# OpenMined/PIR

Measured on NVIDIA B200. Metric: pir_queries_per_sec, higher is better.
Workload: dtype u64

## Files before the change

pir_b200/csrc/context.cu:

```cuda
#include <atomic>
#include <cmath>
#include <cstdio>
#include <cstdlib>
#include <cstring>
#include <map>
#include <memory>
#include <optional>
#include <string>
#include <tuple>
#include <vector>

#include "../../include/pir_b200.h"
#include "behz_host.h"
#include "host_math.h"
#include "kernels.cuh"

using namespace pirb;

namespace {

thread_local std::string g_err;
int fail(int code, const std::string& msg) {
  g_err = msg;
  return code;
// ... 392 lines not shown
    n_rows = (u32)((npt + dimL - 1) / dimL);
    u64 off = compact_rows ? compact_rows : c->dims[0];
    for (int e = 1; e < d - 1; ++e) off += c->dims[e];
    sv_last = d_sv + off * ctL;
  }
  int n_split;
  RC(run_scan(c, sv_last, sv_qstride, n_queries, dimL, n_rows, npt, d >= 2, &n_split, st, svt));
  if (prof) cudaEventRecord(c->ev[3], st);
  if (d == 1) {
    if (partial) {
      LAUNCH(c, launch_modadd_reduce(P, c->part.p, ctL, n_split, d_out, 1, st, n_queries, (u64)n_split * ctL, ctL));
    } else {
      LAUNCH(c, launch_ntt_inv(P, c->part.p, d_out, 2 * k, k, 0, n_split, (u64)n_rows * ctL, n_queries,
                               (u64)n_split * n_rows * ctL, ctL, st));
    }
    if (prof) { cudaEventRecord(c->ev[4], st); cudaEventRecord(c->ev[5], st); }
    return 0;
  }
  RC(c->bufA[0].ensure((size_t)n_queries * n_rows * ctL * sizeof(u64)));
  LAUNCH(c, launch_ntt_inv(P, c->part.p, c->bufA[0].p, (int)(n_rows * 2 * k), k, 0, n_split, (u64)n_rows * ctL,
                           n_queries, (u64)n_split * n_rows * ctL, (u64)n_rows * ctL, st));
  if (prof) cudaEventRecord(c->ev[4], st);
  if (forked) CU(cudaStreamWaitEvent(st, c->ev_join, 0));
  u32 n_entries = n_rows;
  u32 w = 1;
  int cur = 0;
  for (int l = d - 2; l >= 0; --l) {
    const u32 dim = (l == 0) ? (c->top_hi - c->top_lo) : c->dims[l];
    const u32 n_groups = (n_entries + dim - 1) / dim;
    const u32 w_out = w * c->two_er;
    u64 sv_off = (l == 0) ? (compact_rows ? 0 : c->top_lo) : (compact_rows ? compact_rows : c->dims[0]);
    for (int e = 1; e < l; ++e) sv_off += c->dims[e];
    const u64 n_cts_in = (u64)n_entries * w;
    RC(c->pts.ensure((size_t)n_queries * n_cts_in * c->two_er * c->ptL * sizeof(u64)));
    LAUNCH(c, launch_reencode_ntt(P, c->bufA[cur].p, c->pts.p, (int)(n_queries * n_cts_in), st));
    const u32 slices = (u32)(c->ptL / 256);
    const int ns = dim_mac_config(P, (u64)slices * w_out * n_groups * n_queries, dim, c->sm_count);
    RC(c->part.ensure((size_t)n_queries * ns * n_groups * w_out * ctL * sizeof(u64)));
    LAUNCH(c, launch_dim_mac(P, c->pts.p, n_cts_in * c->two_er * c->ptL, d_sv + sv_off * ctL, sv_qstride, n_queries, dim,
                             n_entries, n_groups, w_out, ns, c->part.p, st));
    const u64 lvl_cts = (u64)n_groups * w_out;
    if (l == 0 && partial) {
      LAUNCH(c, launch_modadd_reduce(P, c->part.p, lvl_cts * ctL, ns, d_out, lvl_cts, st, n_queries, (u64)ns * lvl_cts * ctL,
                                     lvl_cts * ctL));
    } else {
      u64* dst = d_out;
      if (l != 0) {
        RC(c->bufA[cur ^ 1].ensure((size_t)n_queries * lvl_cts * ctL * sizeof(u64)));
        dst = c->bufA[cur ^ 1].p;
      }
      LAUNCH(c, launch_ntt_inv(P, c->part.p, dst, (int)(lvl_cts * 2 * k), k, 0, ns, lvl_cts * ctL, n_queries,
                               (u64)ns * lvl_cts * ctL, lvl_cts * ctL, st));
    }
    n_entries = n_groups;
    w = w_out;
    cur ^= 1;
  }
  if (prof) cudaEventRecord(c->ev[5], st);
  return 0;
}

int ct_level(pirb_ctx* c, const u64* key, const u64* A, u64 a_bstride, int s1, const u64* S, u64 s_bstride, u32 dim,
             u32 n_entries, int n_queries, u64* out, u64 out_bstride, cudaStream_t st) {
  pirb_ctx::CtMul& M = c->ct;
  const DevParams& P = c->P;
  const BehzC& B = M.B;
  const int k = c->k, nb = M.nbsk, sp = s1 + 1;
  const u64 N = c->N;
  const u64 ctL = c->ctL;
  const u64 sq_stride = (u64)dim * ctL, sb_stride = (u64)dim * 2 * nb * N;
  RC(M.sq.ensure((size_t)n_queries * sq_stride * sizeof(u64)));
  RC(M.sb.ensure((size_t)n_queries * sb_stride * sizeof(u64)));
  LAUNCH(c, launch_ntt_fwd(P, S, M.sq.p, (int)(dim * 2 * k), k, 0, n_queries, s_bstride, sq_stride, st));
// ... 1410 lines not shown
```

pir_b200/csrc/kernels.cuh:

```cuda
#pragma once
#include <cuda_runtime.h>

#include "pirb_common.h"
#include "tc_plan.h"

namespace pirb {

struct LevelArgs {
  const u64* src_off;
  const u64* dst_off;
  int n_trees;
  int j;
  u32 ginv;
  u32 g;
  u64 q_stride;
  int n_queries;
  const u64* const* key_tab;
  u64* xch;
  u64* dbg;
  int dbg_clock;
};

cudaError_t launch_ntt_fwd(const DevParams& P, const u64* in, u64* out, int n_polys, int cycle, int off,
                           int n_batch, u64 in_bstride, u64 out_bstride, cudaStream_t st);
cudaError_t launch_ntt_inv(const DevParams& P, const u64* in, u64* out, int n_polys, int cycle, int off, int n_parts,
                           u64 part_stride, int n_batch, u64 in_bstride, u64 out_bstride, cudaStream_t st);

cudaError_t launch_db_preprocess(const DevParams& P, const u64* coeffs, u64* out, u64 n_pt, cudaStream_t st);

cudaError_t launch_ks_digits(const DevParams& P, const u64* work, const LevelArgs& L, u64* dig, cudaStream_t st);
cudaError_t launch_ks_mac_intt(const DevParams& P, const u64* dig, const u64* key, u64* acc, int n_nodes,
                               cudaStream_t st, const u64* const* key_tab = nullptr, u32 nodes_per_query = 1);
cudaError_t launch_ks_combine(const DevParams& P, u64* work, const LevelArgs& L, const u64* acc, int mode,
                              cudaStream_t st);

bool ks_cluster_supported(const DevParams& P);
cudaError_t launch_ks_level_cluster(const DevParams& P, u64* work, const LevelArgs& L, const u64* key, int mode,
                                    cudaStream_t st);

cudaError_t launch_mul_inv_pow_x(const DevParams& P, const u64* in, u64* out, u32 kpow, int n_cts, cudaStream_t st);

cudaError_t launch_scan(const DevParams& P, const u64* db, u64 num_pt, u32 dimL, u32 n_rows, const u64* sv,
                        u64 sv_qstride, int n_queries, int n_split, u64* part, cudaStream_t st);
void scan_config(const DevParams& P, u32 dimL, u32 n_rows, int n_queries, int sm_count, int* n_split);

cudaError_t launch_reencode_ntt(const DevParams& P, const u64* cts, u64* pts, int n_cts, cudaStream_t st);

int dim_mac_config(const DevParams& P, u64 base_ctas, u32 len, int sm_count);
cudaError_t launch_dim_mac(const DevParams& P, const u64* pts, u64 pts_qstride, const u64* sv, u64 sv_qstride,
                           int n_queries, u32 dim, u32 n_entries_in, u32 n_groups, u32 w_out, int n_split, u64* part,
                           cudaStream_t st);

cudaError_t launch_modadd_reduce(const DevParams& P, const u64* in, u64 stride, int n_parts, u64* out, u64 n_cts,
                                 cudaStream_t st, int n_batch = 1, u64 in_bstride = 0, u64 out_bstride = 0);
cudaError_t launch_modadd_reduce_ptrs(const DevParams& P, const u64* const* peers_dev, int n_parts, u64 offset_limbs,
                                      u64* out, u64 n_cts, cudaStream_t st);

cudaError_t launch_place_roots(const DevParams& P, const u64* query, u64 query_qstride, u64* work, const u64* root_off,
                               int n_trees, int n_queries, u64 q_stride, cudaStream_t st);

struct PushArgs {
  u64* const* peers;
  u32 n_ranks;
  u32 d0;
  u32 rows_per_rank;
  u64 slot_off;
  u64 g_first;
  u64 dst_qstride;
};
cudaError_t launch_ntt_fwd_push(const DevParams& P, const u64* in, u64 in_qstride, u32 n_entries, u32 n_queries,
                                const PushArgs& A, cudaStream_t st);
cudaError_t launch_push_head(const DevParams& P, const u64* in, u64 in_qstride, u32 n_entries, u32 n_queries,
                             const PushArgs& A, cudaStream_t st);
cudaError_t launch_push_rows(u64* const* peers_dev, u32 n_ranks, const u8* stage, u64 src_stride, u32 seg_bytes, u32 n_segs,
                             u64 dst_off, u64 dst_stride, cudaStream_t st);
cudaError_t launch_signal(u64* const* peers_dev, u32 n_ranks, u64 flag_off_limbs, u64 value, cudaStream_t st);
cudaError_t launch_wait(const u64* flags, u32 n_ranks, u64 value, u64 timeout_ns, u64* err, cudaStream_t st);

struct TcGeom {
// ... 46 lines not shown
```

pir_b200/csrc/kernels_ntt.cu:

```cuda
#include <cstdlib>
#include <set>
#include <type_traits>
#include <utility>

#include "kernels.cuh"
#include "pirb_device.cuh"

namespace pirb {

template <int LOGN>
struct Cfg {
  static constexpr int N = 1 << LOGN;
  static constexpr int NT = (N / 8 < 512) ? N / 8 : 512;
  static constexpr size_t SMEM = sizeof(u64) * N;
  static constexpr int MINB = LOGN <= 13 ? 2 : 1;
};

template <int LOGN, int ENG>
__global__ void __launch_bounds__(Cfg<LOGN>::NT, Cfg<LOGN>::MINB)
k_ntt_fwd(const __grid_constant__ DevParams P, const u64* __restrict__ in, u64* __restrict__ out, int cycle, int off,
          u64 in_bstride, u64 out_bstride) {
  constexpr int N = Cfg<LOGN>::N, NT = Cfg<LOGN>::NT;
  extern __shared__ u64 s[];
  const int tid = threadIdx.x;
// ... 224 lines not shown
           int n_parts, u64 part_stride, u64 in_bstride, u64 out_bstride) {
  constexpr int N = Cfg2<LOGN>::N, NT = Cfg2<LOGN>::NT;
  extern __shared__ u64 s[];
  const int tid = threadIdx.x;
  const int j = blockIdx.x % cycle;
  const u64 p0 = (u64)(blockIdx.x / cycle) * 2 * cycle + j;
  const ModC& m = P.m[j + off];
  double* TW = reinterpret_cast<double*>(s + 2 * N);
  u64* bar = s + 3 * N;
  ntt2_stage_table<LOGN, true>(m, TW, bar, tid);
  const u64* src = in + blockIdx.y * in_bstride + p0 * N;
  u64* dst = out + blockIdx.y * out_bstride + p0 * N;
#pragma unroll
  for (int i = tid; i < N; i += NT) {
    u64 v = src[i], w = src[(u64)cycle * N + i];
    for (int g = 1; g < n_parts; ++g) {
      v = addmod(v, src[g * part_stride + i], m.q);
      w = addmod(w, src[g * part_stride + (u64)cycle * N + i], m.q);
    }
    s[swz(i)] = eng_load<ENG_FP64>(v);
    s[N + swz(i)] = eng_load<ENG_FP64>(w);
  }
  __syncthreads();
  mbar_wait(bar, 0);
  ntt2_inverse<LOGN, NT>(s, TW, m, tid);
#pragma unroll
  for (int i = tid; i < N; i += NT) {
    dst[i] = eng_store_inv<ENG_FP64>(s[swz(i)], i, m);
    dst[(u64)cycle * N + i] = eng_store_inv<ENG_FP64>(s[N + swz(i)], i, m);
  }
}

template <int LOGN>
__global__ void __launch_bounds__(Cfg2<LOGN>::NT, 2)
k_reencode_ntt2(const __grid_constant__ DevParams P, const u64* __restrict__ cts, u64* __restrict__ pts) {
  constexpr int N = Cfg2<LOGN>::N, NT = Cfg2<LOGN>::NT;
  extern __shared__ u64 s[];
  const int tid = threadIdx.x;
  const int jp = blockIdx.z, e0 = blockIdx.y * 2;
  const u64 x = blockIdx.x;
  const int k = P.k;
  const ModC& m = P.m[jp];
  double* TW = reinterpret_cast<double*>(s + 2 * N);
  u64* bar = s + 3 * N;
  ntt2_stage_table<LOGN, false>(m, TW, bar, tid);
  const u64 mask = (u64)((1u << P.ptb) - 1);
  const u64 inc = m.q - P.t;
#pragma unroll
  for (int h = 0; h < 2; ++h) {
    const int e = e0 + h;
    const u64* src = cts + (x * 2 * k + (u64)P.re_poly[e] * k + P.re_mod[e]) * N;
    const u32 shift = P.re_shift[e];
#pragma unroll
    for (int i = tid; i < N; i += NT) {
      const u64 c = (src[i] >> shift) & mask;
      s[h * N + swz(i)] = eng_load<ENG_FP64>(c >= P.thr ? c + inc : c);
    }
  }
  __syncthreads();
  mbar_wait(bar, 0);
  ntt2_forward<LOGN, NT>(s, TW, m, tid);
#pragma unroll
  for (int h = 0; h < 2; ++h) {
    u64* dst = pts + ((x * P.two_er + e0 + h) * k + jp) * N;
#pragma unroll
    for (int i = tid; i < N; i += NT) dst[i] = eng_store_fwd<ENG_FP64>(s[h * N + swz(i)], m);
  }
}

static bool ntt2_ok(const DevParams& P) {
  static const bool off = getenv("PIRB_NTT2") && getenv("PIRB_NTT2")[0] == '0';
  return !off && P.ntt_engine == ENG_FP64 && P.logn <= 12 && P.logn >= 11;
}
template <typename K>
static cudaError_t ensure_smem2(K kernel, size_t bytes);

template <typename K>
static cudaError_t ensure_smem(K kernel, size_t bytes) {
  if (bytes <= 48 * 1024) return cudaSuccess;
  static std::set<std::pair<int, const void*>> configured;
  int dev = 0;
  cudaGetDevice(&dev);
  const auto key = std::make_pair(dev, reinterpret_cast<const void*>(kernel));
  if (configured.count(key)) return cudaSuccess;
  cudaError_t e = cudaFuncSetAttribute(kernel, cudaFuncAttributeMaxDynamicSharedMemorySize, (int)bytes);
  if (e == cudaSuccess) configured.insert(key);
  return e;
}

template <typename K>
static cudaError_t ensure_smem2(K kernel, size_t bytes) { return ensure_smem(kernel, bytes); }

template <int V>
using IntC = std::integral_constant<int, V>;

template <typename F>
static cudaError_t dispatch(const DevParams& P, F&& f) {
#define PIRB_CASE(LN)                                                   \
  case LN:                                                              \
    switch (P.ntt_engine) {                                             \
// ... 74 lines not shown
    kern<<<dim3((unsigned)n_pt, P.k), Cfg<LN>::NT, Cfg<LN>::SMEM, st>>>(P, coeffs, out);
    return cudaGetLastError();
  });
}

cudaError_t launch_ks_digits(const DevParams& P, const u64* work, const LevelArgs& L, u64* dig, cudaStream_t st) {
  const unsigned nodes = (unsigned)L.n_queries * L.n_trees << L.j;
  if (!nodes) return cudaSuccess;
  return dispatch(P, [&](auto ln, auto lz) {
    constexpr int LN = decltype(ln)::value;
    constexpr int LZ = decltype(lz)::value;
    auto kern = k_ks_digits<LN, LZ>;
    cudaError_t e = ensure_smem(kern, Cfg<LN>::SMEM);
    if (e != cudaSuccess) return e;
    kern<<<dim3(nodes, P.k + 1, P.k), Cfg<LN>::NT, Cfg<LN>::SMEM, st>>>(P, work, L, dig);
    return cudaGetLastError();
  });
}

cudaError_t launch_ks_mac_intt(const DevParams& P, const u64* dig, const u64* key, u64* acc, int n_nodes,
                               cudaStream_t st, const u64* const* key_tab, u32 nodes_per_query) {
  if (n_nodes <= 0) return cudaSuccess;
  return dispatch(P, [&](auto ln, auto lz) {
    constexpr int LN = decltype(ln)::value;
    constexpr int LZ = decltype(lz)::value;
    auto kern = k_ks_mac_intt<LN, LZ>;
    cudaError_t e = ensure_smem(kern, Cfg<LN>::SMEM);
    if (e != cudaSuccess) return e;
    kern<<<dim3(n_nodes, P.k + 1, 2), Cfg<LN>::NT, Cfg<LN>::SMEM, st>>>(P, dig, key, acc, key_tab, nodes_per_query);
    return cudaGetLastError();
  });
}

cudaError_t launch_reencode_ntt(const DevParams& P, const u64* cts, u64* pts, int n_cts, cudaStream_t st) {
  if (n_cts <= 0) return cudaSuccess;
  if (ntt2_ok(P) && P.two_er % 2 == 0) {
    auto go2 = [&](auto ln) -> cudaError_t {
      constexpr int LN = decltype(ln)::value;
      auto kern = k_reencode_ntt2<LN>;
      cudaError_t e = ensure_smem2(kern, Cfg2<LN>::SMEM);
      if (e != cudaSuccess) return e;
      kern<<<dim3(n_cts, P.two_er / 2, P.k), Cfg2<LN>::NT, Cfg2<LN>::SMEM, st>>>(P, cts, pts);
      return cudaGetLastError();
    };
    return P.logn == 12 ? go2(IntC<12>{}) : go2(IntC<11>{});
  }
  return dispatch(P, [&](auto ln, auto lz) {
    constexpr int LN = decltype(ln)::value;
    constexpr int LZ = decltype(lz)::value;
    auto kern = k_reencode_ntt<LN, LZ>;
    cudaError_t e = ensure_smem(kern, Cfg<LN>::SMEM);
    if (e != cudaSuccess) return e;
    kern<<<dim3(n_cts, P.two_er, P.k), Cfg<LN>::NT, Cfg<LN>::SMEM, st>>>(P, cts, pts);
    return cudaGetLastError();
  });
}

}
```

pir_b200/csrc/pirb_device.cuh:

```cuda
#pragma once
#include <cuda_runtime.h>

#include "pirb_common.h"

namespace pirb {

__device__ __forceinline__ u64 csub(u64 x, u64 q) { return x >= q ? x - q : x; }
__device__ __forceinline__ u64 addmod(u64 a, u64 b, u64 q) { return csub(a + b, q); }
__device__ __forceinline__ u64 submod(u64 a, u64 b, u64 q) { return a >= b ? a - b : a + q - b; }
__device__ __forceinline__ u64 negmod(u64 a, u64 q) { return a ? q - a : 0; }

__device__ __forceinline__ u64 shoup_lazy(u64 x, u64 w, u64 ws, u64 q) {
  u64 h = __umul64hi(x, ws);
  return x * w - h * q;
}
__device__ __forceinline__ u64 shoup(u64 x, u64 w, u64 ws, u64 q) { return csub(shoup_lazy(x, w, ws, q), q); }

__device__ __forceinline__ void mac128(u64& lo, u64& hi, u64 a, u64 b) {
  u64 pl = a * b, ph = __umul64hi(a, b);
  asm("add.cc.u64 %0, %0, %2;\n\taddc.u64 %1, %1, %3;" : "+l"(lo), "+l"(hi) : "l"(pl), "l"(ph));
}

__device__ __forceinline__ u64 barrett128(u64 lo, u64 hi, u64 q, u64 r_hi, u64 r_lo);
__device__ __forceinline__ double f64_modmul(double y, double w, double wi, double q);
// ... 229 lines not shown
  }
  ntt_inv_pass<LOGN, NT, 0, R0, LAZY>(s, m.irp, m.irps, q, tid);
  __syncthreads();
}

__device__ __forceinline__ u64 canon_fwd(u64 v, const ModC& m, bool lazy) {
  if (lazy) return barrett64(v, m.q, m.ratio_hi);
  v = v >= 2 * m.q ? v - 2 * m.q : v;
  return csub(v, m.q);
}
__device__ __forceinline__ u64 inv_finish(u64 v, const ModC& m) { return shoup(v, m.inv_n, m.inv_n_s, m.q); }

__device__ __forceinline__ double f64_modmul(double y, double w, double wi, double q) {
  const double M = 6755399441055744.0;
  const double h = __dmul_rn(y, w);
  const double l = __fma_rn(y, w, -h);
  const double c = __dadd_rn(__fma_rn(y, wi, M), -M);
  const double r = __fma_rn(-c, q, h);
  return __dadd_rn(r, l);
}
__device__ __forceinline__ double f64_canon(double v, double q, double qinv) {
  const double M = 6755399441055744.0;
  const double c = __dadd_rn(__fma_rn(v, qinv, M), -M);
  double r = __fma_rn(-c, q, v);
  return r < 0.0 ? __dadd_rn(r, q) : r;
}
__device__ __forceinline__ double u64_to_f64_exact(u64 v) {
  return __dadd_rn(__longlong_as_double((long long)(v | 0x4330000000000000ull)), -4503599627370496.0);
}
__device__ __forceinline__ u64 f64_to_u64_exact(double d) {
  return (u64)__double_as_longlong(__dadd_rn(d, 4503599627370496.0)) & 0x000FFFFFFFFFFFFFull;
}

struct TwGlobal {
  const double2* t;
  __device__ __forceinline__ void get(int i, double& w, double& wi) const {
    const double2 v = __ldg(t + i);
    w = v.x;
    wi = v.y;
  }
};
struct TwShared {
  const double* t;
  double qinv;
  __device__ __forceinline__ void get(int i, double& w, double& wi) const {
    w = t[i];
    wi = __dmul_rn(w, qinv);
  }
};

template <int LOGN, int NT, int S0, int R, class TW>
__device__ __forceinline__ void f64_fwd_pass(double* __restrict__ s, const TW tw, double q, int tid) {
  constexpr int N = 1 << LOGN;
  constexpr int E = 1 << R;
  constexpr int TL = N >> (S0 + R);
  constexpr int UNITS = N >> R;
#pragma unroll 1
  for (int u = tid; u < UNITS; u += NT) {
    const int lo = u & (TL - 1);
    const int hi = u / TL;
    const int base = hi * (TL << R) + lo;
    double x[E];
#pragma unroll
    for (int e = 0; e < E; ++e) x[e] = s[swz(base + e * TL)];
#pragma unroll
    for (int a = 0; a < R; ++a) {
      const int half = E >> (a + 1);
      const int mbase = (1 << (S0 + a)) + (hi << a);
#pragma unroll
      for (int b = 0; b < (1 << a); ++b) {
        double w, wi;
        tw.get(mbase + b, w, wi);
#pragma unroll
        for (int c = 0; c < half; ++c) {
          const int e0 = b * 2 * half + c, e1 = e0 + half;
          const double T = f64_modmul(x[e1], w, wi, q);
          x[e1] = __dadd_rn(x[e0], -T);
          x[e0] = __dadd_rn(x[e0], T);
        }
      }
    }
#pragma unroll
    for (int e = 0; e < E; ++e) s[swz(base + e * TL)] = x[e];
  }
}
template <int LOGN, int NT, int S0, int R, class TW>
__device__ __forceinline__ void f64_inv_pass(double* __restrict__ s, const TW iw, double q, int tid) {
  constexpr int N = 1 << LOGN;
  constexpr int E = 1 << R;
  constexpr int TL = N >> (S0 + R);
  constexpr int UNITS = N >> R;
#pragma unroll 1
  for (int u = tid; u < UNITS; u += NT) {
    const int lo = u & (TL - 1);
    const int hi = u / TL;
    const int base = hi * (TL << R) + lo;
    double x[E];
#pragma unroll
    for (int e = 0; e < E; ++e) x[e] = s[swz(base + e * TL)];
#pragma unroll
    for (int a = R - 1; a >= 0; --a) {
      const int dist = E >> (a + 1);
      const int g = dist * TL;
#pragma unroll
      for (int c = 0; c < dist; ++c) {
        double w, wi;
        iw.get(g + c * TL + lo, w, wi);
#pragma unroll
        for (int b = 0; b < (1 << a); ++b) {
          const int e0 = b * 2 * dist + c, e1 = e0 + dist;
          const double T = f64_modmul(x[e1], w, wi, q);
          x[e1] = __dadd_rn(x[e0], -T);
          x[e0] = __dadd_rn(x[e0], T);
        }
      }
    }
#pragma unroll
    for (int e = 0; e < E; ++e) s[swz(base + e * TL)] = x[e];
  }
}

enum { ENG_INT = 0, ENG_INT_LAZY = 1, ENG_FP64 = 2 };

template <int ENG>
__device__ __forceinline__ u64 eng_load(u64 v) {
  if constexpr (ENG == ENG_FP64) return (u64)__double_as_longlong(u64_to_f64_exact(v));
  else return v;
}
template <int ENG>
__device__ __forceinline__ u64 eng_store_fwd(u64 word, const ModC& m) {
  if constexpr (ENG == ENG_FP64) return f64_to_u64_exact(f64_canon(__longlong_as_double((long long)word), m.qd, m.qinv));
  else return canon_fwd(word, m, ENG == ENG_INT_LAZY);
}
template <int ENG>
__device__ __forceinline__ u64 eng_store_inv(u64 word, int i, const ModC& m) {
  if constexpr (ENG == ENG_FP64) {
    const double2 f2 = __ldg(m.fin + i);
    double t = f64_modmul(__longlong_as_double((long long)word), f2.x, f2.y, m.qd);
    t = t < 0.0 ? __dadd_rn(t, m.qd) : t;
    return f64_to_u64_exact(t);
  } else {
    return inv_finish(word, m);
  }
}
__device__ __forceinline__ double f64_addmod(double a, double b, double q) {
  const double s = __dadd_rn(a, b);
  return s >= q ? __dadd_rn(s, -q) : s;
}
__device__ __forceinline__ double f64_submod(double a, double b, double q) {
  const double d = __dadd_rn(a, -b);
  return d < 0.0 ? __dadd_rn(d, q) : d;
// ... 87 lines not shown
```

pir_b200/csrc/kernels_cluster.cu:

```cuda
#include <cooperative_groups.h>

#include <algorithm>
#include <cstdlib>

#include <type_traits>

#include "kernels.cuh"
#include "pirb_device.cuh"

namespace cg = cooperative_groups;

namespace pirb {

template <int LOGN>
struct CCfg {
  static constexpr int N = 1 << LOGN;
  static constexpr int NT = (N / 8 < 512) ? N / 8 : 512;
};

__device__ __forceinline__ u64 mod_down_c(u64 a, u64 last, const DevParams& P, int j, u64 Pq) {
  const ModC& m = P.m[j];
  u64 l = last + P.half_P;
  l = l >= Pq ? l - Pq : l;
  u64 r = submod(barrett64(l, m.q, m.ratio_hi), P.half_P_mod[j], m.q);
// ... 238 lines not shown
    }
  }
  PIRB_STAMP(7);
}

template <int LOGN, int K>
__global__ void __launch_bounds__(CCfg<LOGN>::NT, 2)
k_ks_level_cluster2(const __grid_constant__ DevParams P, u64* __restrict__ work, const LevelArgs L,
                    const u64* __restrict__ key_arg, int mode) {
  constexpr int N = CCfg<LOGN>::N, NT = CCfg<LOGN>::NT;
  constexpr int NB = K < 2 ? 2 : K;
  extern __shared__ u64 smem[];
  cg::cluster_group cluster = cg::this_cluster();
  const int tid = threadIdx.x;
  constexpr int k = K;
  const int I = (int)cluster.block_rank();
  const u32 z = blockIdx.x / (k + 1);
  const u32 kk = z & ((1u << L.j) - 1);
  const u32 tq = z >> L.j;
  const u32 ti = tq % L.n_trees, qi = tq / L.n_trees;
  const u64* __restrict__ key = L.key_tab ? L.key_tab[qi] : key_arg;
  const u64 ctL = (u64)2 * k * N;
  const u64* src = work + qi * L.q_stride + L.src_off[ti] + kk * ctL;
  const ModC& mI = P.m[I];
  const double qd = mI.qd, qinv = mI.qinv;
  double* TWb = reinterpret_cast<double*>(smem + (size_t)NB * N);
  u64* twbar = smem + (size_t)(NB + 1) * N;
  if (tid == 0) {
    mbar_init(twbar, 1);
    asm volatile("fence.mbarrier_init.release.cluster;" ::: "memory");
    mbar_expect_tx(twbar, N * 8);
    bulk_g2s_plain(TWb, mI.fw1, N * 8, twbar);
  }
  asm volatile("griddepcontrol.launch_dependents;");
  {
    constexpr int LINES = N * 8 / 128;
    for (int J = 0; J < k; ++J)
      for (int c = 0; c < 2; ++c) {
        const char* kp = reinterpret_cast<const char*>(key + ((u64)(J * 2 + c) * (k + 1) + I) * N);
        for (int l = tid; l < LINES; l += NT) asm volatile("prefetch.global.L2 [%0];" ::"l"(kp + (size_t)l * 128));
      }
    asm volatile("griddepcontrol.wait;" ::: "memory");
  }
#pragma unroll
  for (int J = 0; J < k; ++J) {
    u64* D = smem + (size_t)J * N;
    const u64* c1 = src + (u64)(k + J) * N;
    const u64 qJ = P.m[J].q;
    const bool need_reduce = qJ > mI.q;
#pragma unroll
    for (int i = tid; i < N; i += NT) {
      u64 v = c1[i];
      const u32 t = ((u32)i * L.g) & (2 * N - 1);
      if (t & N) v = negmod(v, qJ);
      if (need_reduce) v = barrett64(v, mI.q, mI.ratio_hi);
      D[swz(t & (N - 1))] = eng_load<ENG_FP64>(v);
    }
  }
  __syncthreads();
  mbar_wait(twbar, 0);
  {
    constexpr int R0 = ((LOGN - 1) % 3) + 1;
    const TwShared tw{TWb, qinv};
    auto pass_all = [&](auto s0, auto r) {
      constexpr int S0 = decltype(s0)::value, R = decltype(r)::value;
#pragma unroll
      for (int J = 0; J < k; ++J) f64_fwd_pass<LOGN, NT, S0, R>(reinterpret_cast<double*>(smem + (size_t)J * N), tw, qd, tid);
      __syncthreads();
    };
    pass_all(std::integral_constant<int, 0>{}, std::integral_constant<int, R0>{});
    if constexpr (LOGN > R0) pass_all(std::integral_constant<int, R0>{}, std::integral_constant<int, 3>{});
    if constexpr (LOGN > R0 + 3) pass_all(std::integral_constant<int, R0 + 3>{}, std::integral_constant<int, 3>{});
    if constexpr (LOGN > R0 + 6) pass_all(std::integral_constant<int, R0 + 6>{}, std::integral_constant<int, 3>{});
    if constexpr (LOGN > R0 + 9) pass_all(std::integral_constant<int, R0 + 9>{}, std::integral_constant<int, 3>{});
  }
  if (tid == 0) {
    asm volatile("fence.proxy.async.shared::cta;" ::: "memory");
    mbar_expect_tx(twbar, N * 8);
    bulk_g2s_plain(TWb, mI.iw1, N * 8, twbar);
  }
  {
    constexpr int CH = 4;
#pragma unroll 1
    for (int i0 = tid; i0 < N; i0 += CH * NT) {
      double a0[CH], a1[CH];
      int si[CH];
#pragma unroll
      for (int e = 0; e < CH; ++e) { si[e] = swz(i0 + e * NT); a0[e] = 0.0; a1[e] = 0.0; }
#pragma unroll
      for (int J = 0; J < k; ++J) {
        const u64* D = smem + (size_t)J * N;
        const u64* kp0 = key + ((u64)(J * 2 + 0) * (k + 1) + I) * N + i0;
        const u64* kp1 = key + ((u64)(J * 2 + 1) * (k + 1) + I) * N + i0;
        u64 dv[CH], k0[CH], k1[CH];
#pragma unroll
        for (int e = 0; e < CH; ++e) {
          dv[e] = D[si[e]];
          k0[e] = __ldg(kp0 + e * NT);
          k1[e] = __ldg(kp1 + e * NT);
        }
#pragma unroll
        for (int e = 0; e < CH; ++e) {
          const double y = __longlong_as_double((long long)dv[e]);
          const double kd0 = u64_to_f64_exact(k0[e]), kd1 = u64_to_f64_exact(k1[e]);
          a0[e] = __dadd_rn(a0[e], f64_modmul(y, kd0, __dmul_rn(kd0, qinv), qd));
          a1[e] = __dadd_rn(a1[e], f64_modmul(y, kd1, __dmul_rn(kd1, qinv), qd));
        }
      }
#pragma unroll
      for (int e = 0; e < CH; ++e) {
        smem[si[e]] = (u64)__double_as_longlong(a0[e]);
        (smem + N)[si[e]] = (u64)__double_as_longlong(a1[e]);
      }
    }
  }
  __syncthreads();
  mbar_wait(twbar, 1);
  {
    constexpr int R0 = ((LOGN - 1) % 3) + 1;
    const TwShared iw{TWb, qinv};
    auto pass_both = [&](auto s0, auto r) {
      constexpr int S0 = decltype(s0)::value, R = decltype(r)::value;
      f64_inv_pass<LOGN, NT, S0, R>(reinterpret_cast<double*>(smem), iw, qd, tid);
      f64_inv_pass<LOGN, NT, S0, R>(reinterpret_cast<double*>(smem + N), iw, qd, tid);
      __syncthreads();
    };
    if constexpr (LOGN > R0 + 9) pass_both(std::integral_constant<int, R0 + 9>{}, std::integral_constant<int, 3>{});
    if constexpr (LOGN > R0 + 6) pass_both(std::integral_constant<int, R0 + 6>{}, std::integral_constant<int, 3>{});
    if constexpr (LOGN > R0 + 3) pass_both(std::integral_constant<int, R0 + 3>{}, std::integral_constant<int, 3>{});
    if constexpr (LOGN > R0) pass_both(std::integral_constant<int, R0>{}, std::integral_constant<int, 3>{});
    pass_both(std::integral_constant<int, 0>{}, std::integral_constant<int, R0>{});
  }
  if (I == k) {
#pragma unroll
    for (int c = 0; c < 2; ++c) {
      u64* xo = L.xch + ((u64)z * 2 + c) * N;
      const u64* A = smem + (size_t)c * N;
#pragma unroll
      for (int i = tid; i < N; i += NT) xo[i] = eng_finish_inv_native<ENG_FP64>(A[swz(i)], i, mI);
    }
  } else {
#pragma unroll
    for (int c = 0; c < 2; ++c) {
      u64* A = smem + (size_t)c * N;
#pragma unroll
      for (int i = tid; i < N; i += NT) {
        const double2 f2 = __ldg(mI.fin + i);
        A[swz(i)] = (u64)__double_as_longlong(f64_modmul(__longlong_as_double((long long)A[swz(i)]), f2.x, f2.y, qd));
      }
    }
    const u64* sp = src + (u64)I * N;
    u64* SB = reinterpret_cast<u64*>(TWb);
#pragma unroll
    for (int i = tid; i < N; i += NT) SB[i] = sp[i];
  }
  cluster.sync();
  if (I < k) {
    const int j = I;
    const u64 q = mI.q;
    const u64* SB = reinterpret_cast<const u64*>(TWb);
    u64* dstE = work + qi * L.q_stride + L.dst_off[ti] + kk * ctL;
    const u32 s1 = (2 * N - (1u << L.j)) & (2 * N - 1);
    const double Pqd = P.m[k].qd;
    constexpr int CH = 4;
#pragma unroll
    for (int c = 0; c < 2; ++c) {
      const u64* lastA = L.xch + ((u64)z * 2 + c) * N;
      const u64* A = smem + (size_t)c * N;
      const u64* sp1 = src + (u64)(k + j) * N;
#pragma unroll 1
      for (int i0 = tid; i0 < N; i0 += CH * NT) {
        u64 la[CH], av[CH], pv[CH], gv[CH];
#pragma unroll
        for (int e = 0; e < CH; ++e) {
          const int i = i0 + e * NT;
          la[e] = __ldcg(lastA + i);
          av[e] = A[swz(i)];
          gv[e] = (c == 0) ? galois_gather(SB, i, L.ginv, N, q) : 0;
          pv[e] = (mode == 1) ? 0 : (c == 0 ? SB[i] : sp1[i]);
        }
#pragma unroll
        for (int e = 0; e < CH; ++e) {
          const int i = i0 + e * NT;
          double l = __dadd_rn(__longlong_as_double((long long)la[e]), P.half_P_d);
          l = l >= Pqd ? __dadd_rn(l, -Pqd) : l;
          const double dd = __dadd_rn(__dadd_rn(__longlong_as_double((long long)av[e]), -l), P.half_P_mod_d[j]);
          double md = f64_modmul(dd, P.inv_P_d[j], P.inv_P_di[j], qd);
          if (c == 0) md = __dadd_rn(md, u64_to_f64_exact(gv[e]));
          if (mode == 1) {
            dstE[(u64)(c * k + j) * N + i] = f64_to_u64_exact(f64_canon(md, qd, qinv));
          } else {
            const double pd = u64_to_f64_exact(pv[e]);
            dstE[(u64)(c * k + j) * N + i] = f64_to_u64_exact(f64_canon(__dadd_rn(pd, md), qd, qinv));
            const u32 rr = i + s1;
            double d = __dadd_rn(pd, -md);
            if (rr & N) d = -d;
            (dstE + ((u64)ctL << L.j))[(u64)(c * k + j) * N + (rr & (N - 1))] = f64_to_u64_exact(f64_canon(d, qd, qinv));
          }
        }
      }
    }
  }
}

static size_t ks_cluster_smem(int k, int logn, int engine) {
  const bool tws = engine == ENG_FP64 && logn <= 12;
  return (size_t)((k + 1) / 2 + 1 + (tws ? 1 : 0)) * ((size_t)1 << logn) * sizeof(u64) + (tws ? 16 : 0);
}

static bool ks_cluster_fits(int k, int logn, int engine) {
  return 2 * (k + 1) <= 16 && ks_cluster_smem(k, logn, engine) <= 227 * 1024 && logn >= 11 && logn <= 14;
}

bool ks_cluster_supported(const DevParams& P) { return ks_cluster_fits(P.k, P.logn, P.ntt_engine); }

static size_t ks_cluster_smem_max(int logn, int engine) {
  size_t most = 0;
  for (int k = 1; 2 * (k + 1) <= 16; ++k)
    if (ks_cluster_fits(k, logn, engine)) most = std::max(most, ks_cluster_smem(k, logn, engine));
  return most;
}

static bool ks_cluster2_supported(const DevParams& P) {
  return P.ntt_engine == ENG_FP64 && P.logn <= 12 && P.logn >= 11 && P.k <= 2;
}
template <int LN, int K>
static cudaError_t launch_cluster2(const DevParams& P, u64* work, const LevelArgs& L, const u64* key, int mode,
                                   unsigned nodes, cudaStream_t st) {
  auto kern = k_ks_level_cluster2<LN, K>;
  const size_t smem = (size_t)((K < 2 ? 2 : K) + 1) * P.N * sizeof(u64) + 16;
  static bool configured[64] = {};
  int dev = 0;
  cudaGetDevice(&dev);
  if (!configured[dev & 63]) {
    cudaError_t e = cudaFuncSetAttribute(kern, cudaFuncAttributeMaxDynamicSharedMemorySize, (int)smem);
// ... 101 lines not shown
```

Baseline: 1256.

## Fuse plaintext re-encode NTT with dimension MAC into one kernel

Replaces the separate re-encode NTT kernel (which wrote the full plaintext NTT buffer to global memory) and the dim_mac kernel with one fused kernel. Each CTA runs two half-blocks with named barriers; each re-encodes a ciphertext slice, does the forward NTT in fp64 in shared memory, and multiplies-accumulates against the selection vector with lazy fp64 reduction. It removes the large intermediate pts buffer round-trip and one launch per level, at the cost of redoing the NTT for each split, heavier shared memory use and a split count constrained by the fp64 accumulation chain bound.

```diff
diff --git a/pir_b200/csrc/context.cu b/pir_b200/csrc/context.cu
--- a/pir_b200/csrc/context.cu
+++ b/pir_b200/csrc/context.cu
@@ -448,13 +448,21 @@
     u64 sv_off = (l == 0) ? (compact_rows ? 0 : c->top_lo) : (compact_rows ? compact_rows : c->dims[0]);
     for (int e = 1; e < l; ++e) sv_off += c->dims[e];
     const u64 n_cts_in = (u64)n_entries * w;
-    RC(c->pts.ensure((size_t)n_queries * n_cts_in * c->two_er * c->ptL * sizeof(u64)));
-    LAUNCH(c, launch_reencode_ntt(P, c->bufA[cur].p, c->pts.p, (int)(n_queries * n_cts_in), st));
-    const u32 slices = (u32)(c->ptL / 256);
-    const int ns = dim_mac_config(P, (u64)slices * w_out * n_groups * n_queries, dim, c->sm_count);
-    RC(c->part.ensure((size_t)n_queries * ns * n_groups * w_out * ctL * sizeof(u64)));
-    LAUNCH(c, launch_dim_mac(P, c->pts.p, n_cts_in * c->two_er * c->ptL, d_sv + sv_off * ctL, sv_qstride, n_queries, dim,
-                             n_entries, n_groups, w_out, ns, c->part.p, st));
+    int ns;
+    if (reencode_mac_ok(P)) {
+      ns = reencode_mac_config(P, (u64)n_queries * n_groups * (w_out / 2) * k, dim, c->sm_count);
+      RC(c->part.ensure((size_t)n_queries * ns * n_groups * w_out * ctL * sizeof(u64)));
+      LAUNCH(c, launch_reencode_mac(P, c->bufA[cur].p, n_cts_in * ctL, d_sv + sv_off * ctL, sv_qstride, n_queries, dim,
+                                    n_entries, n_groups, w, ns, c->part.p, st));
+    } else {
+      RC(c->pts.ensure((size_t)n_queries * n_cts_in * c->two_er * c->ptL * sizeof(u64)));
+      LAUNCH(c, launch_reencode_ntt(P, c->bufA[cur].p, c->pts.p, (int)(n_queries * n_cts_in), st));
+      const u32 slices = (u32)(c->ptL / 256);
+      ns = dim_mac_config(P, (u64)slices * w_out * n_groups * n_queries, dim, c->sm_count);
+      RC(c->part.ensure((size_t)n_queries * ns * n_groups * w_out * ctL * sizeof(u64)));
+      LAUNCH(c, launch_dim_mac(P, c->pts.p, n_cts_in * c->two_er * c->ptL, d_sv + sv_off * ctL, sv_qstride, n_queries,
+                               dim, n_entries, n_groups, w_out, ns, c->part.p, st));
+    }
     const u64 lvl_cts = (u64)n_groups * w_out;
     if (l == 0 && partial) {
       LAUNCH(c, launch_modadd_reduce(P, c->part.p, lvl_cts * ctL, ns, d_out, lvl_cts, st, n_queries, (u64)ns * lvl_cts * ctL,
diff --git a/pir_b200/csrc/kernels.cuh b/pir_b200/csrc/kernels.cuh
--- a/pir_b200/csrc/kernels.cuh
+++ b/pir_b200/csrc/kernels.cuh
@@ -45,6 +45,12 @@
 void scan_config(const DevParams& P, u32 dimL, u32 n_rows, int n_queries, int sm_count, int* n_split);
 
 cudaError_t launch_reencode_ntt(const DevParams& P, const u64* cts, u64* pts, int n_cts, cudaStream_t st);
+
+bool reencode_mac_ok(const DevParams& P);
+int reencode_mac_config(const DevParams& P, u64 base_ctas, u32 len, int sm_count);
+cudaError_t launch_reencode_mac(const DevParams& P, const u64* cts, u64 cts_qstride, const u64* sv, u64 sv_qstride,
+                                int n_queries, u32 dim, u32 n_entries_in, u32 n_groups, u32 w, int n_split, u64* part,
+                                cudaStream_t st);
 
 int dim_mac_config(const DevParams& P, u64 base_ctas, u32 len, int sm_count);
 cudaError_t launch_dim_mac(const DevParams& P, const u64* pts, u64 pts_qstride, const u64* sv, u64 sv_qstride,
diff --git a/pir_b200/csrc/kernels_ntt.cu b/pir_b200/csrc/kernels_ntt.cu
--- a/pir_b200/csrc/kernels_ntt.cu
+++ b/pir_b200/csrc/kernels_ntt.cu
@@ -280,40 +280,108 @@
 }
 
 template <int LOGN>
-__global__ void __launch_bounds__(Cfg2<LOGN>::NT, 2)
-k_reencode_ntt2(const __grid_constant__ DevParams P, const u64* __restrict__ cts, u64* __restrict__ pts) {
-  constexpr int N = Cfg2<LOGN>::N, NT = Cfg2<LOGN>::NT;
-  extern __shared__ u64 s[];
-  const int tid = threadIdx.x;
-  const int jp = blockIdx.z, e0 = blockIdx.y * 2;
-  const u64 x = blockIdx.x;
+struct CfgF {
+  static constexpr int N = 1 << LOGN;
+  static constexpr int NTH = N / 8;
+  static constexpr int NT = 2 * NTH;
+  static constexpr size_t SMEM = sizeof(u64) * N * 7 + 16;
+  static constexpr int MINB = LOGN <= 11 ? 2 : 1;
+};
+
+template <int NTH>
+__device__ __forceinline__ void bar_half(int h) { asm volatile("bar.sync %0, %1;" ::"r"(1 + h), "n"(NTH) : "memory"); }
+
+template <int LOGN>
+__global__ void __launch_bounds__(CfgF<LOGN>::NT, CfgF<LOGN>::MINB)
+k_reencode_mac(const __grid_constant__ DevParams P, const u64* __restrict__ cts, u64 cts_qstride,
+               const u64* __restrict__ sv, u64 sv_qstride, u32 dim, u32 n_entries_in, u32 n_groups, u32 w, int n_split,
+               u64* __restrict__ part) {
+  constexpr int N = CfgF<LOGN>::N, NTH = CfgF<LOGN>::NTH;
+  constexpr int R0 = ((LOGN - 1) % 3) + 1;
+  static_assert(LOGN == R0 + 9, "four passes, the last one with unit gap 1");
+  extern __shared__ u64 s[];
+  double* TW = reinterpret_cast<double*>(s + 6 * N);
+  u64* bar = s + 7 * N;
+  const int tid = threadIdx.x;
+  const int jp = blockIdx.y;
+  const u32 x0 = blockIdx.x * 2;
+  const u32 split = blockIdx.z % n_split, gq = blockIdx.z / n_split;
+  const u32 g = gq % n_groups, qi = gq / n_groups;
   const int k = P.k;
+  const u64 kN = (u64)k * N, ctL = 2 * kN;
   const ModC& m = P.m[jp];
-  double* TW = reinterpret_cast<double*>(s + 2 * N);
-  u64* bar = s + 3 * N;
   ntt2_stage_table<LOGN, false>(m, TW, bar, tid);
+  const u32 cnt = min(dim, n_entries_in - g * dim);
+  const u32 per = (dim + n_split - 1) / n_split;
+  const u32 i_lo = split * per, i_hi = min(cnt, i_lo + per);
+  const int h = tid / NTH, ht = tid % NTH;
+  const int e = (int)(x0 % P.two_er) + h;
+  const u64* src0 = cts + qi * cts_qstride + ((u64)g * dim * w + x0 / P.two_er) * ctL +
+                    ((u64)P.re_poly[e] * k + P.re_mod[e]) * N + 8 * ht;
+  const u64 wstride = (u64)w * ctL;
+  const u32 shift = P.re_shift[e];
   const u64 mask = (u64)((1u << P.ptb) - 1);
   const u64 inc = m.q - P.t;
-#pragma unroll
-  for (int h = 0; h < 2; ++h) {
-    const int e = e0 + h;
-    const u64* src = cts + (x * 2 * k + (u64)P.re_poly[e] * k + P.re_mod[e]) * N;
-    const u32 shift = P.re_shift[e];
-#pragma unroll
-    for (int i = tid; i < N; i += NT) {
-      const u64 c = (src[i] >> shift) & mask;
-      s[h * N + swz(i)] = eng_load<ENG_FP64>(c >= P.thr ? c + inc : c);
+  u32 v[8];
+  auto fetch = [&](u32 i) {
+    const u64* src = src0 + i * wstride;
+#pragma unroll
+    for (int r = 0; r < 8; r += 2) {
+      const ulonglong2 c = __ldg(reinterpret_cast<const ulonglong2*>(src + r));
+      v[r] = (u32)((c.x >> shift) & mask);
+      v[r + 1] = (u32)((c.y >> shift) & mask);
     }
-  }
+  };
+  double* acc = reinterpret_cast<double*>(s + 2 * N + (u64)h * 2 * N);
+#pragma unroll
+  for (int r = 0; r < 16; ++r) acc[r * NTH + ht] = 0.0;
+  if (i_lo < i_hi) fetch(i_lo);
+  double* own = reinterpret_cast<double*>(s + h * N);
+  const TwShared tw{TW, m.qinv};
+  const u64* svq = sv + qi * sv_qstride + (u64)jp * N + 8 * ht;
   __syncthreads();
   mbar_wait(bar, 0);
-  ntt2_forward<LOGN, NT>(s, TW, m, tid);
-#pragma unroll
-  for (int h = 0; h < 2; ++h) {
-    u64* dst = pts + ((x * P.two_er + e0 + h) * k + jp) * N;
-#pragma unroll
-    for (int i = tid; i < N; i += NT) dst[i] = eng_store_fwd<ENG_FP64>(s[h * N + swz(i)], m);
-  }
+  for (u32 i = i_lo; i < i_hi; ++i) {
+#pragma unroll
+    for (int r = 0; r < 8; ++r) own[swz(8 * ht + r)] = u64_to_f64_exact(v[r] >= P.thr ? v[r] + inc : v[r]);
+    bar_half<NTH>(h);
+    f64_fwd_pass<LOGN, NTH, 0, R0>(own, tw, m.qd, ht);
+    bar_half<NTH>(h);
+    f64_fwd_pass<LOGN, NTH, R0, 3>(own, tw, m.qd, ht);
+    bar_half<NTH>(h);
+    f64_fwd_pass<LOGN, NTH, R0 + 3, 3>(own, tw, m.qd, ht);
+    bar_half<NTH>(h);
+    f64_fwd_pass<LOGN, NTH, R0 + 6, 3>(own, tw, m.qd, ht);
+    const u64* s0 = svq + (u64)i * ctL;
+#pragma unroll
+    for (int p = 0; p < 2; ++p) {
+      u64 sw[8];
+#pragma unroll
+      for (int r = 0; r < 8; r += 2) {
+        const ulonglong2 c = __ldg(reinterpret_cast<const ulonglong2*>(s0 + p * kN + r));
+        sw[r] = c.x;
+        sw[r + 1] = c.y;
+      }
+#pragma unroll
+      for (int r = 0; r < 8; ++r) {
+        const double wv = u64_to_f64_exact(sw[r]);
+        double& a = acc[(p * 8 + r) * NTH + ht];
+        a = f64_modmul_acc(a, own[swz(8 * ht + r)], wv, __dmul_rn(wv, m.qinv), m.qd);
+      }
+    }
+    if (i + 1 < i_hi) fetch(i + 1);
+  }
+  const u64 w_out = (u64)w * P.two_er;
+  u64* o = part + ((((u64)qi * n_split + split) * n_groups + g) * w_out + x0 + h) * ctL + (u64)jp * N + 8 * ht;
+#pragma unroll
+  for (int p = 0; p < 2; ++p)
+#pragma unroll
+    for (int r = 0; r < 8; r += 2) {
+      ulonglong2 c;
+      c.x = f64_to_u64_exact(f64_canon(acc[(p * 8 + r) * NTH + ht], m.qd, m.qinv));
+      c.y = f64_to_u64_exact(f64_canon(acc[(p * 8 + r + 1) * NTH + ht], m.qd, m.qinv));
+      *reinterpret_cast<ulonglong2*>(o + p * kN + r) = c;
+    }
 }
 
 static bool ntt2_ok(const DevParams& P) {
@@ -454,19 +522,56 @@
   });
 }
 
+bool reencode_mac_ok(const DevParams& P) { return ntt2_ok(P); }
+
+int reencode_mac_config(const DevParams& P, u64 base_ctas, u32 len, int sm_count) {
+  int resident = 1;
+  auto probe = [&](auto ln) -> cudaError_t {
+    constexpr int LN = decltype(ln)::value;
+    auto kern = k_reencode_mac<LN>;
+    cudaError_t e = ensure_smem(kern, CfgF<LN>::SMEM);
+    if (e == cudaSuccess) e = cudaOccupancyMaxActiveBlocksPerMultiprocessor(&resident, kern, CfgF<LN>::NT, CfgF<LN>::SMEM);
+    return e;
+  };
+  if ((P.logn == 12 ? probe(IntC<12>{}) : probe(IntC<11>{})) != cudaSuccess || resident < 1) resident = 1;
+  u64 q_max = 0;
+  for (int j = 0; j < P.k; ++j) q_max = std::max(q_max, P.m[j].q);
+  const u32 chain = f64_modmul_chain_max(q_max);
+  const u64 slots = (u64)sm_count * resident;
+  const u32 s_min = (len + chain - 1) / chain;
+  u32 best = s_min > 0 ? s_min : 1;
+  u64 best_cost = ~0ull;
+  for (u32 s = best; s <= std::max<u32>(len, best); ++s) {
+    const u64 waves = (base_ctas * s + slots - 1) / slots;
+    const u64 cost = waves * ((len + s - 1) / s + 1);
+    if (cost < best_cost) best_cost = cost, best = s;
+  }
+  return (int)best;
+}
+
+cudaError_t launch_reencode_mac(const DevParams& P, const u64* cts, u64 cts_qstride, const u64* sv, u64 sv_qstride,
+                                int n_queries, u32 dim, u32 n_entries_in, u32 n_groups, u32 w, int n_split, u64* part,
+                                cudaStream_t st) {
+  if (!n_groups || !n_queries) return cudaSuccess;
+  const dim3 grid((unsigned)w * P.two_er / 2, P.k, (unsigned)n_queries * n_groups * n_split);
+  if (grid.x > 0x7fffffffu || grid.z > 65535) return cudaErrorInvalidConfiguration;
+  u64 q_max = 0;
+  for (int j = 0; j < P.k; ++j) q_max = std::max(q_max, P.m[j].q);
+  if ((dim + n_split - 1) / n_split > f64_modmul_chain_max(q_max)) return cudaErrorInvalidValue;
+  auto go = [&](auto ln) -> cudaError_t {
+    constexpr int LN = decltype(ln)::value;
+    auto kern = k_reencode_mac<LN>;
+    cudaError_t e = ensure_smem(kern, CfgF<LN>::SMEM);
+    if (e != cudaSuccess) return e;
+    kern<<<grid, CfgF<LN>::NT, CfgF<LN>::SMEM, st>>>(P, cts, cts_qstride, sv, sv_qstride, dim, n_entries_in, n_groups, w,
+                                                      n_split, part);
+    return cudaGetLastError();
+  };
+  return P.logn == 12 ? go(IntC<12>{}) : go(IntC<11>{});
+}
+
 cudaError_t launch_reencode_ntt(const DevParams& P, const u64* cts, u64* pts, int n_cts, cudaStream_t st) {
   if (n_cts <= 0) return cudaSuccess;
-  if (ntt2_ok(P) && P.two_er % 2 == 0) {
-    auto go2 = [&](auto ln) -> cudaError_t {
-      constexpr int LN = decltype(ln)::value;
-      auto kern = k_reencode_ntt2<LN>;
-      cudaError_t e = ensure_smem2(kern, Cfg2<LN>::SMEM);
-      if (e != cudaSuccess) return e;
-      kern<<<dim3(n_cts, P.two_er / 2, P.k), Cfg2<LN>::NT, Cfg2<LN>::SMEM, st>>>(P, cts, pts);
-      return cudaGetLastError();
-    };
-    return P.logn == 12 ? go2(IntC<12>{}) : go2(IntC<11>{});
-  }
   return dispatch(P, [&](auto ln, auto lz) {
     constexpr int LN = decltype(ln)::value;
     constexpr int LZ = decltype(lz)::value;
diff --git a/pir_b200/csrc/pirb_device.cuh b/pir_b200/csrc/pirb_device.cuh
--- a/pir_b200/csrc/pirb_device.cuh
+++ b/pir_b200/csrc/pirb_device.cuh
@@ -285,6 +285,15 @@
   return (u64)__double_as_longlong(__dadd_rn(d, 4503599627370496.0)) & 0x000FFFFFFFFFFFFFull;
 }
 
+constexpr double F64_FWD_BOUND = 9.0;
+__host__ __device__ __forceinline__ u32 f64_modmul_chain_max(u64 q) {
+  const double r = 2251799813685248.0 / (0.57 * (double)q);
+  return r >= 1073741824.0 ? 1u << 30 : (u32)r;
+}
+__device__ __forceinline__ double f64_modmul_acc(double acc, double y, double w, double wi, double q) {
+  return __dadd_rn(acc, f64_modmul(y, w, wi, q));
+}
+
 struct TwGlobal {
   const double2* t;
   __device__ __forceinline__ void get(int i, double& w, double& wi) const {
```

Measured after the change: 1217, median of 6. -3.1%, worse.

## Fuse inverse-NTT epilogue scaling and precompute Galois permutation in keyswitch cluster kernel

Applied to the files above, without the earlier changes.

The final-factor scaling, and for the last modulus the exchange-buffer write, are folded into the last inverse NTT pass through a store functor, which removes one extra pass over shared memory. Source limbs are prefetched into L2 after the grid-dependency wait. The Galois automorphism is now applied as a scatter when filling the shared staging buffer, so the mod-down loop reads it directly instead of gathering. That loop is also fully unrolled with CH = N/NT. Timing stamp macros are added, and the heavier unroll may raise register pressure.

```diff
diff --git a/pir_b200/csrc/kernels_cluster.cu b/pir_b200/csrc/kernels_cluster.cu
--- a/pir_b200/csrc/kernels_cluster.cu
+++ b/pir_b200/csrc/kernels_cluster.cu
@@ -294,6 +294,7 @@
     mbar_expect_tx(twbar, N * 8);
     bulk_g2s_plain(TWb, mI.fw1, N * 8, twbar);
   }
+  PIRB_STAMP(0);
   asm volatile("griddepcontrol.launch_dependents;");
   {
     constexpr int LINES = N * 8 / 128;
@@ -303,6 +304,10 @@
         for (int l = tid; l < LINES; l += NT) asm volatile("prefetch.global.L2 [%0];" ::"l"(kp + (size_t)l * 128));
       }
     asm volatile("griddepcontrol.wait;" ::: "memory");
+    if (I < k) {
+      const char* sp = reinterpret_cast<const char*>(src + (u64)I * N);
+      for (int l = tid; l < LINES; l += NT) asm volatile("prefetch.global.L2 [%0];" ::"l"(sp + (size_t)l * 128));
+    }
   }
 #pragma unroll
   for (int J = 0; J < k; ++J) {
@@ -320,6 +325,7 @@
     }
   }
   __syncthreads();
+  PIRB_STAMP(1);
   mbar_wait(twbar, 0);
   {
     constexpr int R0 = ((LOGN - 1) % 3) + 1;
@@ -336,6 +342,7 @@
     if constexpr (LOGN > R0 + 6) pass_all(std::integral_constant<int, R0 + 6>{}, std::integral_constant<int, 3>{});
     if constexpr (LOGN > R0 + 9) pass_all(std::integral_constant<int, R0 + 9>{}, std::integral_constant<int, 3>{});
   }
+  PIRB_STAMP(2);
   if (tid == 0) {
     asm volatile("fence.proxy.async.shared::cta;" ::: "memory");
     mbar_expect_tx(twbar, N * 8);
@@ -377,6 +384,7 @@
     }
   }
   __syncthreads();
+  PIRB_STAMP(3);
   mbar_wait(twbar, 1);
   {
     constexpr int R0 = ((LOGN - 1) % 3) + 1;
@@ -391,78 +399,83 @@
     if constexpr (LOGN > R0 + 6) pass_both(std::integral_constant<int, R0 + 6>{}, std::integral_constant<int, 3>{});
     if constexpr (LOGN > R0 + 3) pass_both(std::integral_constant<int, R0 + 3>{}, std::integral_constant<int, 3>{});
     if constexpr (LOGN > R0) pass_both(std::integral_constant<int, R0>{}, std::integral_constant<int, 3>{});
-    pass_both(std::integral_constant<int, 0>{}, std::integral_constant<int, R0>{});
-  }
-  if (I == k) {
-#pragma unroll
-    for (int c = 0; c < 2; ++c) {
-      u64* xo = L.xch + ((u64)z * 2 + c) * N;
-      const u64* A = smem + (size_t)c * N;
-#pragma unroll
-      for (int i = tid; i < N; i += NT) xo[i] = eng_finish_inv_native<ENG_FP64>(A[swz(i)], i, mI);
-    }
-  } else {
-#pragma unroll
-    for (int c = 0; c < 2; ++c) {
-      u64* A = smem + (size_t)c * N;
-#pragma unroll
-      for (int i = tid; i < N; i += NT) {
-        const double2 f2 = __ldg(mI.fin + i);
-        A[swz(i)] = (u64)__double_as_longlong(f64_modmul(__longlong_as_double((long long)A[swz(i)]), f2.x, f2.y, qd));
-      }
-    }
+    const double2* fin = mI.fin;
+    if (I == k) {
+#pragma unroll
+      for (int c = 0; c < 2; ++c) {
+        u64* xo = L.xch + ((u64)z * 2 + c) * N;
+        f64_inv_pass<LOGN, NT, 0, R0>(reinterpret_cast<double*>(smem + (size_t)c * N), iw, qd, tid,
+                                      [=](double*, int i, double v) {
+                                        const double2 f2 = __ldg(fin + i);
+                                        const double t = f64_modmul(v, f2.x, f2.y, qd);
+                                        xo[i] = (u64)__double_as_longlong(t < 0.0 ? __dadd_rn(t, qd) : t);
+                                      });
+      }
+    } else {
+      const auto scale = [=](double* s, int i, double v) {
+        const double2 f2 = __ldg(fin + i);
+        s[swz(i)] = f64_modmul(v, f2.x, f2.y, qd);
+      };
+      f64_inv_pass<LOGN, NT, 0, R0>(reinterpret_cast<double*>(smem), iw, qd, tid, scale);
+      f64_inv_pass<LOGN, NT, 0, R0>(reinterpret_cast<double*>(smem + N), iw, qd, tid, scale);
+    }
+  }
+  PIRB_STAMP(4);
+  u64* SB = reinterpret_cast<u64*>(TWb);
+  if (I < k) {
     const u64* sp = src + (u64)I * N;
-    u64* SB = reinterpret_cast<u64*>(TWb);
-#pragma unroll
-    for (int i = tid; i < N; i += NT) SB[i] = sp[i];
-  }
+    const u64 q = mI.q;
+    __syncthreads();
+#pragma unroll
+    for (int i = tid; i < N; i += NT) {
+      u64 v = sp[i];
+      const u32 t = ((u32)i * L.g) & (2 * N - 1);
+      if (t & N) v = negmod(v, q);
+      SB[t & (N - 1)] = v;
+    }
+  }
+  PIRB_STAMP(5);
   cluster.sync();
+  PIRB_STAMP(6);
   if (I < k) {
     const int j = I;
-    const u64 q = mI.q;
-    const u64* SB = reinterpret_cast<const u64*>(TWb);
     u64* dstE = work + qi * L.q_stride + L.dst_off[ti] + kk * ctL;
     const u32 s1 = (2 * N - (1u << L.j)) & (2 * N - 1);
     const double Pqd = P.m[k].qd;
-    constexpr int CH = 4;
+    constexpr int CH = N / NT;
 #pragma unroll
     for (int c = 0; c < 2; ++c) {
       const u64* lastA = L.xch + ((u64)z * 2 + c) * N;
       const u64* A = smem + (size_t)c * N;
-      const u64* sp1 = src + (u64)(k + j) * N;
-#pragma unroll 1
-      for (int i0 = tid; i0 < N; i0 += CH * NT) {
-        u64 la[CH], av[CH], pv[CH], gv[CH];
-#pragma unroll
-        for (int e = 0; e < CH; ++e) {
-          const int i = i0 + e * NT;
-          la[e] = __ldcg(lastA + i);
-          av[e] = A[swz(i)];
-          gv[e] = (c == 0) ? galois_gather(SB, i, L.ginv, N, q) : 0;
-          pv[e] = (mode == 1) ? 0 : (c == 0 ? SB[i] : sp1[i]);
-        }
-#pragma unroll
-        for (int e = 0; e < CH; ++e) {
-          const int i = i0 + e * NT;
-          double l = __dadd_rn(__longlong_as_double((long long)la[e]), P.half_P_d);
-          l = l >= Pqd ? __dadd_rn(l, -Pqd) : l;
-          const double dd = __dadd_rn(__dadd_rn(__longlong_as_double((long long)av[e]), -l), P.half_P_mod_d[j]);
-          double md = f64_modmul(dd, P.inv_P_d[j], P.inv_P_di[j], qd);
-          if (c == 0) md = __dadd_rn(md, u64_to_f64_exact(gv[e]));
-          if (mode == 1) {
-            dstE[(u64)(c * k + j) * N + i] = f64_to_u64_exact(f64_canon(md, qd, qinv));
-          } else {
-            const double pd = u64_to_f64_exact(pv[e]);
-            dstE[(u64)(c * k + j) * N + i] = f64_to_u64_exact(f64_canon(__dadd_rn(pd, md), qd, qinv));
-            const u32 rr = i + s1;
-            double d = __dadd_rn(pd, -md);
-            if (rr & N) d = -d;
-            (dstE + ((u64)ctL << L.j))[(u64)(c * k + j) * N + (rr & (N - 1))] = f64_to_u64_exact(f64_canon(d, qd, qinv));
-          }
-        }
-      }
-    }
-  }
+      const u64* spc = src + (u64)(c * k + j) * N;
+      u64 la[CH], pv[CH];
+#pragma unroll
+      for (int e = 0; e < CH; ++e) {
+        la[e] = __ldcg(lastA + tid + e * NT);
+        pv[e] = (mode == 1) ? 0 : spc[tid + e * NT];
+      }
+#pragma unroll
+      for (int e = 0; e < CH; ++e) {
+        const int i = tid + e * NT;
+        double l = __dadd_rn(__longlong_as_double((long long)la[e]), P.half_P_d);
+        l = l >= Pqd ? __dadd_rn(l, -Pqd) : l;
+        const double dd = __dadd_rn(__dadd_rn(__longlong_as_double((long long)A[swz(i)]), -l), P.half_P_mod_d[j]);
+        double md = f64_modmul(dd, P.inv_P_d[j], P.inv_P_di[j], qd);
+        if (c == 0) md = __dadd_rn(md, u64_to_f64_exact(SB[i]));
+        if (mode == 1) {
+          dstE[(u64)(c * k + j) * N + i] = f64_to_u64_exact(f64_canon(md, qd, qinv));
+        } else {
+          const double pd = u64_to_f64_exact(pv[e]);
+          dstE[(u64)(c * k + j) * N + i] = f64_to_u64_exact(f64_canon(__dadd_rn(pd, md), qd, qinv));
+          const u32 rr = i + s1;
+          double d = __dadd_rn(pd, -md);
+          if (rr & N) d = -d;
+          (dstE + ((u64)ctL << L.j))[(u64)(c * k + j) * N + (rr & (N - 1))] = f64_to_u64_exact(f64_canon(d, qd, qinv));
+        }
+      }
+    }
+  }
+  PIRB_STAMP(7);
 }
 
 static size_t ks_cluster_smem(int k, int logn, int engine) {
diff --git a/pir_b200/csrc/pirb_device.cuh b/pir_b200/csrc/pirb_device.cuh
--- a/pir_b200/csrc/pirb_device.cuh
+++ b/pir_b200/csrc/pirb_device.cuh
@@ -337,8 +337,11 @@
     for (int e = 0; e < E; ++e) s[swz(base + e * TL)] = x[e];
   }
 }
-template <int LOGN, int NT, int S0, int R, class TW>
-__device__ __forceinline__ void f64_inv_pass(double* __restrict__ s, const TW iw, double q, int tid) {
+struct PassStore {
+  __device__ __forceinline__ void operator()(double* s, int i, double v) const { s[swz(i)] = v; }
+};
+template <int LOGN, int NT, int S0, int R, class TW, class ST = PassStore>
+__device__ __forceinline__ void f64_inv_pass(double* __restrict__ s, const TW iw, double q, int tid, const ST st = ST{}) {
   constexpr int N = 1 << LOGN;
   constexpr int E = 1 << R;
   constexpr int TL = N >> (S0 + R);
@@ -369,7 +372,7 @@
       }
     }
 #pragma unroll
-    for (int e = 0; e < E; ++e) s[swz(base + e * TL)] = x[e];
+    for (int e = 0; e < E; ++e) st(s, base + e * TL, x[e]);
   }
 }
 
```

Result: no change. 1256 before, 1267 after, median of 6 (+0.8%).
